# jacobwilliams/splpak

Hardware: AMD Instinct MI355X
Metric: fitted points/sec (splcw) + evals/sec (splfe), 3-D 1e7 pts 64^3 nodes (higher is better)
Workload: dtype f64; 1 GPU; C3: 3-D splcw least-squares spline fit, 10000000 weighted scattered points (Park-Miller stream, seed 42), 64x64x64 nodes, xtrap=1, real64; ncol=262144, points_per_gpu=10000000, points_total=10000000, parallelism=single GPU, rccl_ranks=0, refine_steps=2

## Files before the change

splpak_amd/csrc/ndchol.hip:

```cpp
#include "ndstate.hpp"
#include <cstdlib>

namespace splpak {
namespace nd {

hipError_t nd_prefit(splpak_plan *p, hipStream_t st, void *user)
{
    NdState *s = static_cast<NdState *>(user);
    s->tail_pending = false;
    if (s->sch.staged_init && !s->dist) return hipSuccess;
    if (!s->str.sU || !s->ev.evPre || splpak::opt_get("SPLPAK_ND_NO_EARLY_CLEAR")) return hipSuccess;
    long long head = 0;
    if (p->gscratch == s->factor) head = p->gscratch_doubles < s->factor_doubles ? p->gscratch_doubles : s->factor_doubles;
    else if (p->gscratch >= s->factor && p->gscratch < s->factor + s->factor_doubles) return hipSuccess;
    if (head >= s->factor_doubles) return hipSuccess;
    hipError_t e = hipEventRecord(s->ev.evPre, st);
    if (e == hipSuccess) e = hipStreamWaitEvent(s->str.sU, s->ev.evPre, 0);
    const int clear_wgs = splpak::opt_get("SPLPAK_ND_CLEAR_WGS") ? atoi(splpak::opt_get("SPLPAK_ND_CLEAR_WGS")) : 128;
    if (e == hipSuccess) {
        if (clear_wgs > 0) {
            launch_clear(clear_wgs, s->factor + head, s->factor_doubles - head, s->str.sU);
            e = hipGetLastError();
        } else
            e = hipMemsetAsync(s->factor + head, 0, sizeof(double) * (size_t)(s->factor_doubles - head), s->str.sU);
    }
    if (e == hipSuccess) e = hipEventRecord(s->ev.evTail, s->str.sU);
    if (e != hipSuccess) return e;
    s->tail_pending = true;
    s->head_doubles = head;
    return hipSuccess;
}

hipError_t nd_assemble(splpak_plan *p, hipStream_t st, void *user)
{
    NdState *s = static_cast<NdState *>(user);
    hipError_t e = hipSuccess;
    if (s->sch.staged_init && !s->dist) {
        if (!s->sch.istarts.empty())
            for (int x : s->sch.istarts[0]) launch_init(s, p->g, p->nst, s->fac.init.l[(size_t)x][0], st);
        return hipGetLastError();
    }
    if (s->tail_pending) {
        if (s->head_doubles > 0) e = hipMemsetAsync(s->factor, 0, sizeof(double) * (size_t)s->head_doubles, st);
        if (e == hipSuccess) e = hipStreamWaitEvent(st, s->ev.evTail, 0);
        s->tail_pending = false;
    } else
        e = hipMemsetAsync(s->factor, 0, sizeof(double) * (size_t)s->factor_doubles, st);
    if (e != hipSuccess) return e;
    launch_assemble(s, p->g, p->nst, st);
    return hipGetLastError();
}

namespace {

struct FactorRun {
    splpak_plan *p;
    NdState *s;
    hipStream_t st, sP, sU, sR;
    int *info_dev;
    double *minpiv_dev;
    CholStats *stats;
    bool timing;
    int pin_rounds;
    int qnext = 0;
    int la_evt = -1;
    bool joined = false, comm_failed = false;
    void syrk(const JobTable<SyrkJob> &tab, const Launch &l, hipStream_t q, bool schur, bool pinned) { launch_syrk(s, tab, l, q, stats, timing, schur, pinned, qnext); }
    void begin();
    void dist_join();
    void potrf_step(const Launch &lp, int k, hipStream_t sC, bool reserved, hipEvent_t after);
    void stage_prep(int i);
    void chain_step(int stg, int k, bool pinned, bool pin_potrf, int prep);
    void root_stage(int stg);
    void run_stage(int i);
    hipError_t end();
};

void hop(hipEvent_t e, hipStream_t from, hipStream_t to) { (void)hipEventRecord(e, from); (void)hipStreamWaitEvent(to, e, 0); }

void zero_block(NdState *s, int x, hipStream_t q) { launch_zero(s->fac.zero, s->fac.zero.l[(size_t)x][0], q); }

void ensure_events(NdState *s, int steps)
{
    for (auto *v : {&s->ev.evT, &s->ev.evI, &s->ev.evW})
        while ((int)v->size() < steps) v->push_back(nd_event(s));
}

void FactorRun::begin()
{
    NdTree &t = s->t;
    if (timing) {
        if (!s->ev.f0) { s->ev.f0 = nd_event(s, true); s->ev.f1 = nd_event(s, true); }
        (void)hipEventRecord(s->ev.f0, st);
    }
    if (s->used && s->ev.evDone) (void)hipStreamWaitEvent(st, s->ev.evDone, 0);
    if (s->zlast_valid) (void)hipStreamWaitEvent(st, s->ev.evZlast, 0);
    if (!s->s_clean && !s->sch.sc.st.empty())
        for (int x : s->sch.starts[0]) zero_block(s, x, st);
    s->s_clean = false;
    if (s->queues) (void)hipMemsetAsync(s->queues, 0, sizeof(int) * ND_QSTRIDE * (size_t)s->nqueues, st);
    if (s->dist && s->sh.rank != 0)
        for (int id : t.by_depth[(size_t)(s->sh.dcut - 1)]) {
            const NdFront &f = t.fr[(size_t)id];
            (void)hipMemsetAsync(s->factor + s->poff[(size_t)id], 0, sizeof(double) * (size_t)(f.ld * f.wp), st);
        }
    (void)hipEventRecord(s->ev.ev0, st);
    for (hipStream_t q : {sP, sU})
        if (q != st) (void)hipStreamWaitEvent(q, s->ev.ev0, 0);
    if (sR) (void)hipStreamWaitEvent(sR, s->ev.ev0, 0);
}

void FactorRun::dist_join()
{
    NdTree &t = s->t;
    joined = true;
    for (hipStream_t q : {sP, sU, sR})
        if (q) (void)hipStreamSynchronize(q);
    double *scratch = s->sh.join_scratch;
    long long scap = s->sh.join_scratch_doubles;
    if (!s->sch.sc.packed) {
        const double mine_missing = scratch ? 0.0 : 1.0;
        double any_missing = 0.0;
        (void)hipMemcpyAsync(s->part + 1, &mine_missing, sizeof(double), hipMemcpyHostToDevice, st);
        if (plan_allreduce(p, s->part + 1, 1, st) != 0) comm_failed = true;
        (void)hipMemcpyAsync(&any_missing, s->part + 1, sizeof(double), hipMemcpyDeviceToHost, st);
        (void)hipStreamSynchronize(st);
        if (any_missing != 0.0) scap = 0;
    }
    for (int id : t.by_depth[(size_t)(s->sh.dcut - 1)]) {
        const NdFront &f = t.fr[(size_t)id];
        if (plan_allreduce(p, s->factor + s->poff[(size_t)id], f.ld * (long long)f.wp, st) != 0) comm_failed = true;
        if (f.hp == 0) continue;
        const int nt = f.hp / 64;
        const long long tiles = trapezoid_items(nt, nt);
        if (s->sch.sc.packed) {
            if (plan_allreduce(p, s_ptr(s, id), nd_schur_doubles(f, true), st) != 0) comm_failed = true;
        } else if (tiles * 4096 <= scap) {
            launch_tripack(true, s_ptr(s, id), f.lds, nt, scratch, st);
            if (plan_allreduce(p, scratch, tiles * 4096, st) != 0) comm_failed = true;
            launch_tripack(false, s_ptr(s, id), f.lds, nt, scratch, st);
        } else if (plan_allreduce(p, s_ptr(s, id), f.lds * (long long)f.hp, st) != 0)
            comm_failed = true;
    }
    (void)hipStreamSynchronize(st);
}

void FactorRun::potrf_step(const Launch &lp, int k, hipStream_t sC, bool reserved, hipEvent_t after)
{
    if (!reserved) { launch_potrf(s, s->fac.potrf, lp, sC, info_dev, minpiv_dev); return; }
    if (after) (void)hipStreamWaitEvent(sR, after, 0);
    else hop(s->ev.evR0, sC, sR);
    launch_potrf(s, s->fac.potrf, lp, sR, info_dev, minpiv_dev);
    hop(s->ev.evI[(size_t)k], sR, sC);
}

void FactorRun::stage_prep(int i)
{
    for (int x : s->sch.starts[(size_t)i]) zero_block(s, x, sU);
    if (s->sch.staged_init && !s->dist)
        for (int x : s->sch.istarts[(size_t)i]) {
            launch_init(s, p->g, p->nst, s->fac.init.l[(size_t)x][0], sU);
            if (s->sch.sc.st[(size_t)x].dep < 0 && sU != sP) (void)hipEventRecord(s->ev.evP[(size_t)x], sU);
        }
}

void FactorRun::chain_step(int stg, int k, bool pinned, bool pin_potrf, int prep)
{
    FactorTables &F = s->fac;
    const size_t S = (size_t)stg, K = (size_t)k;
    hipStream_t sC = sP;
    const Launch &ls = F.schur.l[S][K], &lf0 = F.fin[0].l[S][K], &lf1 = F.fin[1].l[S][K];
    const bool ahead = pinned && k > 0 && la_evt == k - 1;
    potrf_step(F.potrf.l[S][K], k, sC, pinned && (pin_potrf || ahead), ahead ? s->ev.evW[(size_t)(k - 1)] : nullptr);
    launch_trsm(F.trsm, F.trsm.l[S][K], sC);
    if (prep >= 0) {
        hop(s->ev.evU, sC, sU);
        stage_prep(prep);
    }
    if ((ls.count || lf0.count || lf1.count) && sU != sC) hop(s->ev.evT[K], sC, sU);
    syrk(F.upd, F.upd.l[S][K], sC, false, pinned);
    if (s->sch.chain_la[S] && F.updr.l[S][K].count) {
        if (pinned) {
            (void)hipEventRecord(s->ev.evW[K], sC);
            la_evt = k;
        }
        syrk(F.updr, F.updr.l[S][K], sC, false, pinned);
    }
    syrk(F.updo, F.updo.l[S][K], sC, false, pinned);
    syrk(F.schur, ls, sU, true, pinned);
    syrk(F.fin[0], lf0, sU, true, pinned);
    syrk(F.fin[1], lf1, sU, true, pinned);
}

void FactorRun::root_stage(int stg)
{
    FactorTables &F = s->fac;
    const size_t S = (size_t)stg;
    const int steps = (int)F.potrf.l[S].size();
    ensure_events(s, steps);
    const bool pinned = sR != nullptr && s->nres > 0 && steps > 0 && (int)F.potrf.l[S][0].grid <= pin_rounds * s->nres;
    const bool la = s->sch.lookahead[S] != 0, la2 = s->sch.lookahead[S] == 2;
    for (int k = 0; k < steps; ++k) {
        if (!la) { chain_step(stg, k, pinned, true, -1); continue; }
        const size_t K = (size_t)k;
        const Launch &ltb = F.trsmb.l[S][K], &lur = F.updr.l[S][K];
        potrf_step(F.potrf.l[S][K], k, sP, pinned, nullptr);
        if (ltb.count) {
            if (sU != sP) {
                if (!pinned) (void)hipEventRecord(s->ev.evI[K], sP);
                (void)hipStreamWaitEvent(sU, s->ev.evI[K], 0);
            }
            launch_trsm(F.trsmb, ltb, sU);
        }
        if (!la2 && k > 0 && sU != sP) (void)hipStreamWaitEvent(sP, s->ev.evW[K - 1], 0);
        launch_trsm(F.trsm, F.trsm.l[S][K], sP);
        if (lur.count && sU != sP) hop(s->ev.evT[K], sP, sU);
        if (la2 && k > 0 && sU != sP) (void)hipStreamWaitEvent(sP, s->ev.evW[K - 1], 0);
        syrk(F.upd, F.upd.l[S][K], sP, false, pinned);
        syrk(F.updr, lur, sU, false, pinned);
        if (sU != sP) (void)hipEventRecord(s->ev.evW[K], sU);
    }
    if (sU != sP) hop(s->ev.evU, sU, sP);
}

void FactorRun::run_stage(int i)
{
    FactorTables &F = s->fac;
    const NdStage &S = s->sch.sc.st[(size_t)i];
    if (s->dist && !joined && S.depth <= s->sh.dcut - 1) dist_join();
    auto passes = [&](int k) { return F.schur.l[(size_t)i][(size_t)k].count || F.fin[0].l[(size_t)i][(size_t)k].count || F.fin[1].l[(size_t)i][(size_t)k].count; };
    const int steps = (int)F.potrf.l[(size_t)i].size();
    const bool prep_late = splpak::opt_get("SPLPAK_ND_PREP_EARLY") == nullptr;
    const bool defer = prep_late && i > 0 && i != s->sch.root_stage && sU != sP && steps >= 2 && !passes(0);
    if (i > 0) {
        if (!defer) stage_prep(i);
        if (s->sch.staged_init && !s->dist && S.dep < 0 && sU != sP) (void)hipStreamWaitEvent(sP, s->ev.evP[(size_t)i], 0);
    }
    if (s->sch.fused && S.dep >= 0 && sU != sP) (void)hipStreamWaitEvent(sP, s->ev.evF[(size_t)S.dep], 0);
    la_evt = -1;
    if (i == s->sch.root_stage) { root_stage(i); return; }
    ensure_events(s, steps);
    const bool pinned = sR != nullptr && s->nres > 0 && steps > 0 && ((int)F.potrf.l[(size_t)i][0].grid <= pin_rounds * s->nres || s->sch.chain_la[(size_t)i]);
    const bool unpin_first = splpak::opt_get("SPLPAK_ND_PIN_FIRST") == nullptr;
    bool pass_running = !unpin_first;
    for (int k = 0; k < steps; ++k) {
        chain_step(i, k, pinned, pass_running, k == 0 && defer ? i : -1);
        if (passes(k)) pass_running = true;
    }
    if (s->sch.fused) (void)hipEventRecord(s->ev.evF[(size_t)i], sU);
    else {
        if (sU != sP) hop(s->ev.evU, sU, sP);
        for (int sl = 0; sl < 2; ++sl) launch_add(F.add, F.add.l[(size_t)i][(size_t)sl], sP);
        (void)hipEventRecord(s->ev.evE[(size_t)i], sP);
        if (sU != sP) (void)hipStreamWaitEvent(sU, s->ev.evE[(size_t)i], 0);
    }
}

hipError_t FactorRun::end()
{
    if (s->dist && !joined && s->sh.dcut >= 1) dist_join();
    hipError_t top_err = hipSuccess;
    if (s->mdist) {
        ++s->top.fgen;
        top_err = nd_top_factor(s, st, info_dev, minpiv_dev, stats, timing);
    }
    if (top_err == hipSuccess && !s->sch.sc.st.empty())
        for (int x : s->sch.starts[0]) zero_block(s, x, sU);
    launch_trinv(s->fac.trinv.dev, s->fac.ntrinv, sP);
    (void)hipEventRecord(s->ev.evJ, sP);
    if (sP != st) (void)hipStreamWaitEvent(st, s->ev.evJ, 0);
    if (s->mdist && top_err == hipSuccess) top_err = nd_top_pivots(s, st, info_dev, minpiv_dev);
    if (s->dist) {
        launch_flag(info_dev, s->part, st);
        if (plan_allreduce(p, s->part, 1, st) != 0) comm_failed = true;
        launch_unflag(info_dev, s->part, st);
    }
    if (sU != st) {
        (void)hipEventRecord(s->ev.evZlast, sU);
        s->zlast_valid = true;
    }
    s->s_clean = true;
    (void)hipEventRecord(s->ev.evDone, st);
    s->used = true;
    hipError_t err = hipGetLastError();
    if (timing) {
        (void)hipEventRecord(s->ev.f1, st);
        (void)hipEventSynchronize(s->ev.f1);
        float ms = 0;
        (void)hipEventElapsedTime(&ms, s->ev.f0, s->ev.f1);
        stats->factor_ms = ms;
        for (size_t i = 0; i < (size_t)stats->syrk_launches; ++i) {
            if (hipEventElapsedTime(&ms, s->ev.evA[i], s->ev.evB[i]) == hipSuccess) stats->syrk_ms += ms;
            else (void)hipGetLastError();
        }
    }
    if (err != hipSuccess || top_err != hipSuccess) s->s_clean = false;
    if (comm_failed) return hipErrorUnknown;
    return top_err != hipSuccess ? top_err : err;
}

}

hipError_t nd_factor(splpak_plan *p, int *info_dev, double *minpiv_dev, hipStream_t st, void *user)
{
    NdState *s = static_cast<NdState *>(user);
    const bool timing = p->stats.enabled;
    p->stats = CholStats{};
    p->stats.enabled = timing;
    const bool serial = splpak::opt_get("SPLPAK_NO_LOOKAHEAD") != nullptr;
    FactorRun r{p, s, st, s->str.sP, s->str.sU, s->str.sR, info_dev, minpiv_dev, &p->stats, timing};
    if (serial) r.sP = r.sU = st;
    if (serial || splpak::opt_get("SPLPAK_NO_PANEL_CU")) r.sR = nullptr;
    r.pin_rounds = splpak::opt_get("SPLPAK_ND_PIN_ROUNDS") ? atoi(splpak::opt_get("SPLPAK_ND_PIN_ROUNDS")) : 1;
    r.begin();
    for (int i = 0; i < (int)s->sch.sc.st.size(); ++i) r.run_stage(i);
    return r.end();
}

hipError_t nd_solve(splpak_plan *p, double *x, double *tmp, hipStream_t st, void *user)
{
    (void)tmp;
    NdState *s = static_cast<NdState *>(user);
    NdTree &t = s->t;
    SolveTables &T = s->sol;
    const long long n = t.vec_doubles;
    launch_gather(n, s->rowsrc, x, s->V, st);
    bool comm_failed = false;
    if (s->dist && s->sh.rank != 0)
        for (int id : t.by_depth[(size_t)(s->sh.dcut - 1)]) {
            const NdFront &f = t.fr[(size_t)id];
            (void)hipMemsetAsync(s->V + f.vofs, 0, sizeof(double) * (size_t)f.fp, st);
        }
    const int dlow = s->mdist ? s->top.pt.dcut : 0;
    if (s->mdist) ++s->top.sgen;
    for (int d = t.maxdepth; d >= dlow; --d) {
        if (d < t.maxdepth)
            for (int sl = 0; sl < 2; ++sl) launch_map(T.map, T.map.l[(size_t)(d + 1)][(size_t)sl], false, st);
        if (s->dist && d == s->sh.dcut - 1)
            for (int id : t.by_depth[(size_t)d]) {
                const NdFront &f = t.fr[(size_t)id];
                if (plan_allreduce(p, s->V + f.vofs, f.fp, st) != 0) comm_failed = true;
            }
        const int steps = (int)T.mv.l[(size_t)d].size();
        for (int k = 0; k < steps; ++k) {
            launch_mv(T.mv, T.mv.l[(size_t)d][(size_t)k], st);
            launch_fwd(T.fwd, T.fwd.l[(size_t)d][(size_t)k], st);
        }
    }
    if (s->mdist) {
        hipError_t e = nd_top_forward(s, st);
        if (e == hipSuccess) e = nd_top_backward(s, st);
        if (e != hipSuccess) return e;
    }
    for (int d = dlow; d <= t.maxdepth; ++d) {
        if (d >= 1 && d > dlow) launch_map(T.map, T.map.l[(size_t)d][2], true, st);
        const int steps = (int)T.mv.l[(size_t)d].size();
        for (int k = steps - 1; k >= 0; --k) {
            launch_dot(T.dot, T.dot.l[(size_t)d][(size_t)k], st);
            launch_bwd(T.bwd, T.bwd.l[(size_t)d][(size_t)k], st);
        }
    }
    if (s->dist || s->mdist) {
        (void)hipMemsetAsync(x, 0, sizeof(double) * (size_t)p->g.ncol, st);
        launch_scatter(n, s->sh.rowsrc_out, s->V, x, st);
        if (plan_allreduce(p, x, p->g.ncol, st) != 0) comm_failed = true;
    } else
        launch_scatter(n, s->rowsrc, s->V, x, st);
    if (comm_failed) return hipErrorUnknown;
    return hipGetLastError();
}

}
}
```

splpak_amd/csrc/ndjobs.hip:

```cpp
#include "ndstate.hpp"
#include <algorithm>

namespace splpak {
namespace nd {

namespace {

void front_step_jobs(NdState *s, int stg, int id, int k, bool two_level)
{
    NdTree &t = s->t;
    FactorTables &F = s->fac;
    const NdFront &f = t.fr[(size_t)id];
    const bool la = s->sch.lookahead[(size_t)stg] != 0, la2 = s->sch.lookahead[(size_t)stg] == 2, cla = s->sch.chain_la[(size_t)stg] != 0;
    const int schur_kb = s->sch.schur_kb;
    const int g0 = (k / schur_kb) * schur_kb, gend = std::min(g0 + schur_kb, f.nsteps) - 1;
    double *panel = s->factor + s->poff[(size_t)id];
    double *diag = panel + (long long)k * 256 + (long long)k * 256 * f.ld;
    double *below = diag + 256;
    const int nrows = f.fp - (k + 1) * 256;
    double *i16 = s->inv16 + (long long)(s->lblk[(size_t)id] + k) * 4096;
    const int ncols = std::max(1, std::min(256, f.w - k * 256));
    F.potrf.push(PotrfJob{diag, i16, f.ld, f.own0 + k * 256, ncols});
    const int nc = (f.wp - (k + 1) * 256) / 64, nr = nrows / 64;
    if (nrows > 0) {
        const int ntop = (la && !la2 && nc > 0) ? std::min(nrows, 256) : nrows;
        F.trsm.push(TrsmJob{diag, below, i16, f.ld, ntop, 0, (ncols + 15) / 16, 0}, ntop / 16);
        if (nrows > ntop) F.trsmb.push(TrsmJob{diag, below + ntop, i16, f.ld, nrows - ntop, 0, (ncols + 15) / 16, 0}, (nrows - ntop) / 16);
    }
    if (nc > 0) {
        const SyrkJob proto{below, below + (long long)256 * f.ld, f.ld, f.ld, 0, 0, 0, 1, 64, 0, nullptr, nullptr, nullptr, 0, 0, 0, 0};
        auto trapezoid = [&](JobTable<SyrkJob> &tab, int c, int r) {
            SyrkJob a = proto;
            a.nc = c; a.nr = r;
            tab.push(a, trapezoid_items(c, r));
        };
        auto split = [&](JobTable<SyrkJob> &rect_tab, int nin) {
            const int n4 = std::min(nin, 4);
            trapezoid(F.upd, n4, std::min(nr, 4));
            if (nr > 4) {
                SyrkJob r = proto;
                r.nc = n4; r.nr = nr; r.zinit = -4;
                rect_tab.push(r, (long long)n4 * (nr - 4));
            }
            if (nin > 4) {
                SyrkJob t2 = proto;
                t2.P = below + 256;
                t2.C = below + (long long)256 * f.ld + 256 + (long long)256 * f.ld;
                t2.nc = nin - 4; t2.nr = nr - 4;
                F.updr.push(t2, trapezoid_items(nin - 4, nr - 4));
            }
        };
        if (!la && two_level) {
            const int nc_in = std::min(nc, (gend - k) * 4);
            if (nc_in > 0 && cla) split(F.updr, nc_in);
            else if (nc_in > 0) trapezoid(F.upd, nc_in, nr);
            if (k == gend) {
                SyrkJob o = proto;
                o.P = panel + (long long)(k + 1) * 256 + (long long)g0 * 256 * f.ld;
                o.kb = k - g0 + 1;
                o.nc = nc; o.nr = nr;
                F.updo.push(o, trapezoid_items(nc, nr));
                F.updo.cur.flop += 2.0 * 64 * 64 * 256.0 * o.kb * (double)trapezoid_items(nc, nr);
            }
        } else if (!la)
            trapezoid(F.upd, nc, nr);
        else
            split(la2 ? F.upd : F.updr, nc);
    }
    const int ns = f.hp / 64;
    if (ns > 0 && k == gend) {
        const int kb = k - g0 + 1;
        const int ksl = (k == f.nsteps - 1) ? 4 * ((ncols + 15) / 16) : 64;
        const double jitems = (double)trapezoid_items(ns, ns) - (s->full_diag ? 0.0 : 0.375 * ns);
        const double jflop = 2.0 * 64 * 64 * (256.0 * (kb - 1) + 4.0 * ksl) * jitems;
        const bool boundary = s->mdist && f.depth == s->top.pt.dcut;
        if (s->sch.fused && k == f.nsteps - 1 && f.parent >= 0 && !boundary) {
            const NdFront &pf = t.fr[(size_t)f.parent];
            const int leaf = s->sch.needs[(size_t)id] ? 0 : 1;
            F.fin[f.slot].push(SyrkJob{panel + f.wp + (long long)g0 * 256 * f.ld, s_ptr(s, id), f.ld, s_ld(s, id), ns, ns, 0, kb, ksl, leaf, s->pmap + f.bofs,
                                       s->factor + s->poff[(size_t)f.parent], s_ptr(s, f.parent), pf.ld, s_ld(s, f.parent), pf.wp, f.h},
                               trapezoid_items(ns, ns));
            F.fin[f.slot].cur.flop += jflop;
        } else {
            F.schur.push(SyrkJob{panel + f.wp + (long long)g0 * 256 * f.ld, s_ptr(s, id), f.ld, s_ld(s, id), ns, ns, 0, kb, ksl, 0, nullptr, nullptr, nullptr, 0, 0, 0, 0},
                         trapezoid_items(ns, ns));
            F.schur.cur.flop += jflop;
        }
    }
}

bool stage_jobs(NdState *s, int stg)
{
    NdTree &t = s->t;
    FactorTables &F = s->fac;
    const std::vector<int> &ids = s->sch.sc.st[(size_t)stg].ids;
    F.zero.open();
    for (int id : ids) {
        const NdFront &f = t.fr[(size_t)id];
        if (f.hp == 0 || !s->sch.needs[(size_t)id]) continue;
        const int nt = f.hp / 64;
        F.zero.push(ZeroJob{s_ptr(s, id), s_ld(s, id), nt, 0}, trapezoid_items(nt, nt));
    }
    if (!F.zero.close((size_t)stg, 0)) return false;
    F.init.open();
    for (int id : ids)
        if (s->poff[(size_t)id] >= 0) F.init.push(InitJob{id, 0}, t.fr[(size_t)id].wp);
    if (!F.init.close((size_t)stg, 0)) return false;
    if (s->sch.sc.st[(size_t)stg].depth >= 1 && !s->sch.fused)
        for (int sl = 0; sl < 2; ++sl) {
            F.add.open();
            for (int id : ids) {
                const NdFront &f = t.fr[(size_t)id];
                if (f.slot != sl || f.h == 0) continue;
                const NdFront &p = t.fr[(size_t)f.parent];
                const int nt = f.hp / 64;
                F.add.push(AddJob{s_ptr(s, id), s->pmap + f.bofs, s->factor + s->poff[(size_t)f.parent], s_ptr(s, f.parent), s_ld(s, id), p.ld,
                                  s_ld(s, f.parent), f.h, nt, p.wp, 0},
                           trapezoid_items(nt, nt));
            }
            if (!F.add.close((size_t)stg, (size_t)sl)) return false;
        }
    return true;
}

bool nd_build_factor_jobs(NdState *s)
{
    NdTree &t = s->t;
    FactorTables &F = s->fac;
    const int nstage = (int)s->sch.sc.st.size();
    JobTable<SyrkJob> *const syrk[] = {&F.upd, &F.updr, &F.updo, &F.schur, &F.fin[0], &F.fin[1]};
    s->sch.lookahead.assign((size_t)nstage, 0);
    s->sch.chain_la.assign((size_t)nstage, 0);
    for_each_table(F, [&](auto &tab) { tab.l.assign((size_t)nstage, {}); });
    const bool two_level = splpak::opt_get("SPLPAK_ND_NO_OUTER") == nullptr;
    for (int stg = 0; stg < nstage; ++stg) {
        const std::vector<int> &ids = s->sch.sc.st[(size_t)stg].ids;
        int steps = 0;
        for (int id : ids) steps = std::max(steps, t.fr[(size_t)id].nsteps);
        bool any_schur = false;
        for (int id : ids) any_schur = any_schur || t.fr[(size_t)id].hp > 0;
        const bool la = !any_schur && steps >= 4 && !splpak::opt_get("SPLPAK_ND_NO_ROOT_LOOKAHEAD");
        const bool la2 = la && !(splpak::opt_get("SPLPAK_ND_ROOT_LA") && atoi(splpak::opt_get("SPLPAK_ND_ROOT_LA")) == 1);
        const int cla_blocks = splpak::opt_get("SPLPAK_ND_CHAIN_LA") ? atoi(splpak::opt_get("SPLPAK_ND_CHAIN_LA")) : 8;
        const bool cla = !la && two_level && steps >= 2 && (int)ids.size() <= cla_blocks && !s->mdist;
        s->sch.chain_la[(size_t)stg] = cla ? 1 : 0;
        s->sch.lookahead[(size_t)stg] = la ? (la2 ? 2 : 1) : 0;
        for (int k = 0; k < steps; ++k) {
            F.potrf.open(); F.trsm.open(); F.trsmb.open();
            for (auto *tab : syrk) tab->open();
            for (int id : ids)
                if (k < t.fr[(size_t)id].nsteps) front_step_jobs(s, stg, id, k, two_level);
            const size_t S = (size_t)stg, K = (size_t)k;
            if (!F.potrf.close(S, K) || !F.trsm.close(S, K) || !F.trsmb.close(S, K)) return false;
            for (auto *tab : syrk)
                if (!tab->close(S, K)) return false;
            F.upd.l[S][K].flop = 2.0 * 64 * 64 * 256 * (double)F.upd.l[S][K].grid;
            F.updr.l[S][K].flop = 2.0 * 64 * 64 * 256 * (double)F.updr.l[S][K].grid;
        }
        if (!stage_jobs(s, stg)) return false;
    }
    for (size_t id = 0; id < t.fr.size(); ++id) {
        const NdFront &f = t.fr[id];
        if (!s->mine.empty() && !s->mine[id]) continue;
        for (int k = 0; k < f.nsteps; ++k) {
            const double *diag = s->factor + s->poff[id] + (long long)k * 256 + (long long)k * 256 * f.ld;
            const long long lb = s->lblk[id] + k;
            F.trinv.host.push_back(TrinvJob{diag, s->inv16 + lb * 4096, s->dinv + lb * 65536, s->dinvt + lb * 65536, f.ld});
        }
    }
    F.ntrinv = (int)F.trinv.host.size();
    return true;
}

bool nd_build_solve_jobs(NdState *s)
{
    NdTree &t = s->t;
    SolveTables &T = s->sol;
    const int nd = t.maxdepth + 1;
    for_each_table(T, [&](auto &tab) { tab.l.assign((size_t)nd, {}); });
    long long part_max = 0;
    for (int d = 0; d < nd; ++d) {
        std::vector<int> ids;
        for (int id : t.by_depth[(size_t)d])
            if (s->mine.empty() || s->mine[(size_t)id]) ids.push_back(id);
        int steps = 0;
        for (int id : ids) steps = std::max(steps, t.fr[(size_t)id].nsteps);
        for (int k = 0; k < steps; ++k) {
            T.mv.open(); T.fwd.open(); T.dot.open(); T.bwd.open();
            long long partofs = 0;
            for (int id : ids) {
                const NdFront &f = t.fr[(size_t)id];
                if (k >= f.nsteps) continue;
                const double *below = s->factor + s->poff[(size_t)id] + (long long)k * 256 + (long long)k * 256 * f.ld + 256;
                const int nrows = f.fp - (k + 1) * 256;
                double *Vf = s->V + f.vofs, *Yf = s->Y + f.vofs;
                T.mv.push(MvJob{s->dinv + (long long)(s->lblk[(size_t)id] + k) * 65536, Vf + k * 256, Yf + k * 256});
                int nsplit = 0;
                double *partp = s->part + partofs;
                if (nrows > 0) {
                    T.fwd.push(FwdJob{below, Yf + k * 256, Vf + (k + 1) * 256, f.ld, nrows, 0}, nrows / 64);
                    nsplit = (nrows + DOT_RPS - 1) / DOT_RPS;
                    T.dot.push(DotJob{below, Vf + (k + 1) * 256, partp, f.ld, nrows, nsplit, DOT_RPS, 0}, 16 * nsplit);
                    partofs += (long long)nsplit * 256;
                }
                T.bwd.push(BwdJob{s->dinvt + (long long)(s->lblk[(size_t)id] + k) * 65536, Yf + k * 256, partp, Vf + k * 256, nsplit, 0});
            }
            part_max = std::max(part_max, partofs);
            const size_t D = (size_t)d, K = (size_t)k;
            if (!T.mv.close(D, K) || !T.fwd.close(D, K) || !T.dot.close(D, K) || !T.bwd.close(D, K)) return false;
        }
        if (d >= 1) {
            for (int sl = 0; sl < 2; ++sl) {
                T.map.open();
                for (int id : ids) {
                    const NdFront &f = t.fr[(size_t)id];
                    if (f.slot != sl || f.h == 0) continue;
                    const NdFront &p = t.fr[(size_t)f.parent];
                    T.map.push(MapJob{s->V + f.vofs + f.wp, s->V + p.vofs, s->pmap + f.bofs, f.h, 0});
                }
                if (!T.map.close((size_t)d, (size_t)sl)) return false;
            }
            const int first = T.map.l[(size_t)d][0].first, both = T.map.l[(size_t)d][0].count + T.map.l[(size_t)d][1].count;
            T.map.l[(size_t)d].push_back(Launch{first, both, (unsigned)both, 0});
        }
    }
    return part_max <= s->part_cap;
}

}

int nd_make_jobs(NdState *s)
{
    auto each = [&](auto &&f) { for_each_table(s->fac, f); for_each_table(s->sol, f); };
    each([](auto &tab) { tab.host.clear(); });
    if (!nd_build_factor_jobs(s) || !nd_build_solve_jobs(s)) return SPLPAK_E_UNSUPPORTED;
    bool ok = true;
    each([&](auto &tab) { nd_free_dev(s, &tab.dev); ok = ok && nd_upload(s, &tab.dev, tab.host); });
    return ok ? 0 : SPLPAK_E_NOMEM;
}

bool nd_build_top_jobs(NdState *s)
{
    NdGroup *g = s->grp;
    NdTree &t = s->t;
    Top &T = s->top;
    const NdPartition &pt = T.pt;
    const int me = s->mrank, nseq = pt.nseq;
    const size_t ntop = pt.top.size();
    for_each_table(T, [&](auto &tab) { tab.l.assign(1, std::vector<Launch>((size_t)nseq + 1)); });
    T.rslot.assign((size_t)nseq + 1, -1);
    for (int sl = 0; sl < 2; ++sl) {
        T.l_pull[sl].assign(ntop, Launch());
        T.l_mapf[sl].assign(ntop, -1);
// ... 123 lines not shown
```

splpak_amd/csrc/ndstate.hpp:

```cpp
#pragma once
#include "plan.hpp"
#include "ndtree.hpp"
#include <atomic>
#include <memory>
#include <string>
#include <vector>

namespace splpak {

struct NdGroup {
    int R = 1, chunk = 1;
    std::vector<void *> st;
    std::atomic<int> *abort = nullptr;
    std::atomic<int> own_abort{0};
    HostBarrier bar;
    int nseq = 0;
    std::unique_ptr<std::atomic<int>[]> posted, fposted, bposted, subdone;
    std::vector<int> h_info;
    std::vector<double> h_minpiv;
    bool finalized = false;
    int gen = 0;
};

namespace nd {

struct PotrfJob { double *A; double *inv16; long long ld; int k0; int ncols; };
struct TrsmJob { const double *L; double *X; const double *inv16; long long ld; int nrows; int wg0; int ncb; int pad; };
struct SyrkJob {
    const double *P; double *C; long long ldp, ldc; int nc, nr; int item0; int kb; int ksl; int zinit;
    const int *pm; double *Pp; double *Sp; long long ldpp, ldsp; int wpp; int h;
};
struct ZeroJob { double *S; long long lds; int nt; int tile0; };
struct InitJob { int front; int col0; };
struct TrinvJob { const double *L; const double *inv16; double *dinv; double *dinvt; long long ld; };
struct AddJob { const double *S; const int *pm; double *P; double *Sp; long long lds, ldp, ldsp; int h, nt, wpp, tile0; };
struct MvJob { const double *M; const double *v; double *out; };
struct FwdJob { const double *L; const double *y; double *v; long long ld; int nrows; int wg0; };
struct DotJob { const double *L; const double *x; double *part; long long ld; int nrows; int nsplit; int rps; int wg0; };
struct BwdJob { const double *Mt; const double *y; const double *part; double *x; int nsplit; int pad; };
struct MapJob { double *child; double *par; const int *pm; int h; int pad; };
struct FrontDev { long long panel_off, ld, bofs; int own0, w, wp, h; int top; int pad; };
struct TopColDev { long long off, ld; };
struct PullJob { const double *src; long long lds; const int *pm; double *dst; long long ldd; int c0, c1, h, row0, tile0, ntr, ntc, pad; };

constexpr int DOT_RPS = 1024;
constexpr int ND_QSTRIDE = 16;

inline int *first_item(TrsmJob &j) { return &j.wg0; }
inline int *first_item(SyrkJob &j) { return &j.item0; }
inline int *first_item(ZeroJob &j) { return &j.tile0; }
inline int *first_item(InitJob &j) { return &j.col0; }
inline int *first_item(AddJob &j) { return &j.tile0; }
inline int *first_item(FwdJob &j) { return &j.wg0; }
inline int *first_item(DotJob &j) { return &j.wg0; }
inline int *first_item(PullJob &j) { return &j.tile0; }
template <typename J> inline int *first_item(J &) { return nullptr; }
template <typename J> inline J end_job(const J *) { return J{}; }
inline InitJob end_job(const InitJob *) { return InitJob{-1, 0}; }

struct Launch { int first = 0, count = 0; unsigned grid = 0; double flop = 0; };

template <typename J>
struct JobTable {
    std::vector<J> host;
    J *dev = nullptr;
    std::vector<std::vector<Launch>> l;
    Launch cur;
    long long items = 0;

    void open() { cur = Launch(); cur.first = (int)host.size(); items = 0; }
    void push(J j, long long n = 1)
    {
        if (int *f = first_item(j)) *f = (int)items;
        host.push_back(j);
        items += n;
        ++cur.count;
    }
    bool close(Launch &out, bool sentinel = true)
    {
        if (items > 0x7fffffffLL) { set_error("nested dissection: launch too large"); return false; }
        cur.grid = (unsigned)items;
        J e = end_job((const J *)nullptr);
        if (int *f = first_item(e); f && sentinel && cur.count) { *f = (int)items; host.push_back(e); }
        out = cur;
        return true;
    }
    bool close(size_t r, size_t c, bool sentinel = true)
    {
        if (l[r].size() <= c) l[r].resize(c + 1);
        return close(l[r][c], sentinel);
    }
};

struct FactorTables {
    JobTable<PotrfJob> potrf;
    JobTable<TrsmJob> trsm, trsmb;
    JobTable<SyrkJob> upd;
    JobTable<SyrkJob> updr;
    JobTable<SyrkJob> updo;
    JobTable<SyrkJob> fin[2];
    JobTable<SyrkJob> schur;
    JobTable<TrinvJob> trinv;
    JobTable<AddJob> add;
    JobTable<ZeroJob> zero;
    JobTable<InitJob> init;
    int ntrinv = 0;
};
template <typename F> void for_each_table(FactorTables &T, F &&f)
{
    f(T.potrf); f(T.trsm); f(T.trsmb); f(T.upd); f(T.updr); f(T.updo); f(T.fin[0]); f(T.fin[1]); f(T.schur); f(T.trinv); f(T.add); f(T.zero); f(T.init);
}

struct SolveTables {
    JobTable<MvJob> mv;
    JobTable<FwdJob> fwd;
    JobTable<DotJob> dot;
    JobTable<BwdJob> bwd;
    JobTable<MapJob> map;
};
template <typename F> void for_each_table(SolveTables &T, F &&f) { f(T.mv); f(T.fwd); f(T.dot); f(T.bwd); f(T.map); }

struct Schedule {
    NdSchedule sc;
    std::vector<char> needs;
    std::vector<std::vector<int>> starts;
    std::vector<std::vector<int>> istarts;
    int root_stage = -1;
    int schur_kb = 4;
    std::vector<char> lookahead;
    std::vector<char> chain_la;
    bool fused = true;
    bool staged_init = false;
};

struct Streams {
    hipStream_t sP = nullptr, sU = nullptr, sR = nullptr, sCopy = nullptr;
};

struct Events {
    std::vector<hipEvent_t> all;
    hipEvent_t ev0 = nullptr, evJ = nullptr, evU = nullptr, evZlast = nullptr, evDone = nullptr, evPre = nullptr, evTail = nullptr, evR0 = nullptr;
    hipEvent_t f0 = nullptr, f1 = nullptr;
    std::vector<hipEvent_t> evF;
    std::vector<hipEvent_t> evE;
    std::vector<hipEvent_t> evP;
    std::vector<hipEvent_t> evI;
    std::vector<hipEvent_t> evT;
    std::vector<hipEvent_t> evW;
    std::vector<hipEvent_t> evA, evB;
};

struct Shard {
    int world = 1, rank = 0, dcut = 0;
    double *join_scratch = nullptr;
    long long join_scratch_doubles = 0;
    int *rowsrc_out = nullptr;
};

struct Top {
    NdPartition pt;
    std::vector<long long> tbase;
    std::vector<TopColDev> topcol;
    std::vector<int> toplblk;
    TopColDev *topcol_dev = nullptr;
    double *pbuf[3] = {nullptr, nullptr, nullptr};
    double *stagev = nullptr;
    long long stagev_doubles = 0;
    JobTable<PotrfJob> potrf;
    JobTable<TrsmJob> trsm;
    JobTable<SyrkJob> chain, bulk;
    JobTable<PullJob> pull;
    JobTable<TrinvJob> trinv;
    JobTable<MvJob> mv;
    JobTable<FwdJob> fwd;
    JobTable<DotJob> dot;
    JobTable<BwdJob> bwd;
    JobTable<MapJob> mapf, mapb, maps;
    std::vector<Launch> l_pull[2];
    std::vector<int> l_mapf[2], l_mapb, l_maps;
    std::vector<int> subroots;
    std::vector<int> rslot;
    std::vector<hipEvent_t> evReady, evArr, evCol, evBulk, evSF, evSB, evAdd;
    hipEvent_t evSub = nullptr, evTop = nullptr;
    int fgen = 0, sgen = 0;
};
template <typename F> void for_each_table(Top &T, F &&f)
{
    f(T.potrf); f(T.trsm); f(T.chain); f(T.bulk); f(T.pull); f(T.trinv); f(T.mv); f(T.fwd); f(T.dot); f(T.bwd); f(T.mapf); f(T.mapb); f(T.maps);
}

struct NdState {
    NdTree t;
    int device = 0;
    std::string desc;
    double *factor = nullptr, *dinv = nullptr, *dinvt = nullptr, *inv16 = nullptr;
    long long factor_doubles = 0;
    int nblocks = 0;
    std::vector<char> mine;
    std::vector<long long> poff;
    std::vector<int> lblk;
    double *sarena = nullptr;
    long long sarena_doubles = 0;
    double *V = nullptr, *Y = nullptr, *part = nullptr;
    long long part_cap = 0;
    int *pos = nullptr, *front_of = nullptr, *bpos = nullptr, *pmap = nullptr, *rowsrc = nullptr;
    int *ipos = nullptr;
    std::vector<int> rowsrc_host;
    long long *padwhere = nullptr;
    int npad = 0;
    FrontDev *fdev = nullptr;
    std::vector<void *> owned;
    size_t owned_bytes = 0;
    unsigned *resmap = nullptr;
    int nres = 0;
    int potrf_waves = 8;
    int xmode = 1;
    int full_diag = 0;
    bool small_queue = false;
    int wg4 = 0;
    int small_grid = 1024;
    int *queues = nullptr;
    int nqueues = 0;
    Schedule sch;
    FactorTables fac;
    SolveTables sol;
    Streams str;
    Events ev;
    bool dist = false;
    Shard sh;
    bool mdist = false;
    NdGroup *grp = nullptr;
// ... 75 lines not shown
```

splpak_amd/csrc/options.hip:

```cpp
#include "options.hpp"

#include <cctype>
#include <cstdlib>
#include <cstring>
#include <mutex>

extern char **environ;

namespace splpak {

namespace {
struct Known { const char *name; int documented; };
const Known KNOWN[] = {
    {"SPLPAK_BIN_ATOMIC", 0},
    {"SPLPAK_DEBUG", 1},
    {"SPLPAK_DEBUG_NO_PEER", 0},
    {"SPLPAK_DEBUG_SUMS", 0},
    {"SPLPAK_DEBUG_TWOEND", 0},
    {"SPLPAK_DIST_CHUNK", 0},
    {"SPLPAK_GRAM_SCRATCH_MB", 1},
    {"SPLPAK_GRAM_VALU", 0},
    {"SPLPAK_MPLAN_BAND", 0},
    {"SPLPAK_MPLAN_RCCL", 1},
    {"SPLPAK_NARROW_BW", 0},
    {"SPLPAK_ND", 1},
    {"SPLPAK_ND_CHAIN_LA", 0},
    {"SPLPAK_ND_CHUNK", 0},
    {"SPLPAK_ND_CLEAR_WGS", 0},
    {"SPLPAK_ND_CUT", 1},
    {"SPLPAK_ND_DIST", 0},
    {"SPLPAK_ND_FULL_DIAG", 0},
    {"SPLPAK_ND_HALVES", 0},
    {"SPLPAK_ND_KB", 1},
    {"SPLPAK_ND_NO_EARLY_CLEAR", 0},
    {"SPLPAK_ND_NO_FUSE", 0},
    {"SPLPAK_ND_NO_OUTER", 0},
    {"SPLPAK_ND_NO_ROOT_LOOKAHEAD", 0},
    {"SPLPAK_ND_PIN_FIRST", 0},
    {"SPLPAK_ND_PIN_ROUNDS", 0},
    {"SPLPAK_ND_POTRF_WAVES", 0},
    {"SPLPAK_ND_PREP_EARLY", 0},
    {"SPLPAK_ND_RES_CUS", 1},
    {"SPLPAK_ND_ROOT_LA", 0},
    {"SPLPAK_ND_SMALL_GRID", 0},
    {"SPLPAK_ND_SMALL_QUEUE", 0},
    {"SPLPAK_ND_SPLIT", 1},
    {"SPLPAK_ND_SQUARE", 0},
    {"SPLPAK_ND_STAGED_INIT", 0},
    {"SPLPAK_ND_WG4", 0},
    {"SPLPAK_ND_XCD", 0},
    {"SPLPAK_NO_LOOKAHEAD", 0},
    {"SPLPAK_NO_PANEL_CU", 0},
    {"SPLPAK_NO_PLAN_CACHE", 1},
    {"SPLPAK_NO_REORDER", 1},
    {"SPLPAK_NO_TWOEND", 0},
    {"SPLPAK_PCG_ALWAYS", 0},
    {"SPLPAK_PCG_ASSEMBLE", 0},
    {"SPLPAK_PCG_EAGER", 0},
    {"SPLPAK_PCG_MAXIT", 1},
    {"SPLPAK_PCG_NO_BLOCKS", 0},
    {"SPLPAK_PCG_NO_PAIRS", 0},
    {"SPLPAK_PCG_PAIRS_VALU", 0},
    {"SPLPAK_PCG_TOL1", 1},
    {"SPLPAK_PCG_TOL2", 1},
    {"SPLPAK_PIN_BW", 0},
    {"SPLPAK_RCCL_JOB", 0},
    {"SPLPAK_RCCL_LIB", 1},
    {"SPLPAK_RCCL_ONE_RANK_CALLS", 0},
    {"SPLPAK_RESIDUAL_CELLS", 0},
    {"SPLPAK_ROWS_ONE_STREAM", 0},
    {"SPLPAK_ROWS_TILES", 0},
    {"SPLPAK_SOLVER", 1},
    {"SPLPAK_VIRTUAL_GPUS", 0},
};
std::mutex g_mu;
std::map<std::string, std::string> g_defaults;
thread_local const Options *t_current = nullptr;
thread_local Options t_fallback;
thread_local unsigned long long t_fallback_gen = ~0ull;
unsigned long long g_gen = 0;
}

bool option_canonical(const char *name, std::string &canon)
{
    if (!name) return false;
    std::string s(name);
    for (char &c : s) c = (char)std::toupper((unsigned char)c);
    if (s.rfind("SPLPAK_", 0) != 0) s = "SPLPAK_" + s;
    for (const Known &k : KNOWN)
        if (s == k.name) { canon = s; return true; }
    return false;
}

Options options_snapshot()
{
    Options o;
    for (char **e = environ; e && *e; ++e) {
        if (std::strncmp(*e, "SPLPAK_", 7) != 0) continue;
        const char *eq = std::strchr(*e, '=');
        if (!eq) continue;
        o.kv[std::string(*e, (size_t)(eq - *e))] = std::string(eq + 1);
    }
    std::lock_guard<std::mutex> lk(g_mu);
    for (const auto &d : g_defaults) o.kv[d.first] = d.second;
    return o;
}

int options_set_default(const char *name, const char *value)
{
    std::string canon;
    if (!option_canonical(name, canon)) return -1;
    std::lock_guard<std::mutex> lk(g_mu);
    ++g_gen;
    if (value) g_defaults[canon] = value;
    else g_defaults.erase(canon);
    return 0;
}

const char *opt_get(const char *canon)
{
    if (t_current) return t_current->get(canon);
    unsigned long long gen;
    {
        std::lock_guard<std::mutex> lk(g_mu);
        gen = g_gen;
        auto d = g_defaults.find(canon);
        if (d != g_defaults.end()) {
            if (t_fallback_gen != gen) { t_fallback.kv.clear(); t_fallback_gen = gen; }
            t_fallback.kv[canon] = d->second;
            return t_fallback.kv[canon].c_str();
        }
// ... 9 lines not shown
```

Baseline: 40.66 million points/s.

## Add deeper root look-ahead, pinned group stages, and per-stage triangular inverses

Adds a third root look-ahead form that splits each step's trailing update into a small critical corner (upd), a near-panel column band (updc) and the far remainder (updr). This lets the next potrf wait only on the corner update, through a new per-step event, instead of the whole trailing update. It also pins more multi-step stages to the reserved compute units, and launches triangular-inverse jobs per stage right after each stage factors rather than in one tail batch. A host-side coverage check verifies the split tiles exactly once; the costs are more launches and more event traffic.

```diff
diff --git a/splpak_amd/csrc/ndchol.hip b/splpak_amd/csrc/ndchol.hip
--- a/splpak_amd/csrc/ndchol.hip
+++ b/splpak_amd/csrc/ndchol.hip
@@ -53,6 +53,8 @@
 
 namespace {
 
+constexpr bool PIN_GROUPS_DEFAULT = true, TRINV_STAGED_DEFAULT = true;
+
 struct FactorRun {
     splpak_plan *p;
     NdState *s;
@@ -62,6 +64,8 @@
     CholStats *stats;
     bool timing;
     int pin_rounds;
+    bool pin_groups = false;
+    bool trinv_staged = false;
     int qnext = 0;
     int la_evt = -1;
     bool joined = false, comm_failed = false;
@@ -82,7 +86,7 @@
 
 void ensure_events(NdState *s, int steps)
 {
-    for (auto *v : {&s->ev.evT, &s->ev.evI, &s->ev.evW})
+    for (auto *v : {&s->ev.evT, &s->ev.evI, &s->ev.evW, &s->ev.evD})
         while ((int)v->size() < steps) v->push_back(nd_event(s));
 }
 
@@ -199,11 +203,25 @@
     const int steps = (int)F.potrf.l[S].size();
     ensure_events(s, steps);
     const bool pinned = sR != nullptr && s->nres > 0 && steps > 0 && (int)F.potrf.l[S][0].grid <= pin_rounds * s->nres;
-    const bool la = s->sch.lookahead[S] != 0, la2 = s->sch.lookahead[S] == 2;
+    const bool la = s->sch.lookahead[S] != 0, la2 = s->sch.lookahead[S] == 2, la3 = s->sch.lookahead[S] == 3;
     for (int k = 0; k < steps; ++k) {
         if (!la) { chain_step(stg, k, pinned, true, -1); continue; }
         const size_t K = (size_t)k;
         const Launch &ltb = F.trsmb.l[S][K], &lur = F.updr.l[S][K];
+        if (la3) {
+            const bool ahead = pinned && k > 0 && F.upd.l[S][K - 1].count != 0;
+            potrf_step(F.potrf.l[S][K], k, sP, pinned, ahead ? s->ev.evD[K - 1] : nullptr);
+            launch_trsm(F.trsm, F.trsm.l[S][K], sP);
+            syrk(F.upd, F.upd.l[S][K], sP, false, pinned);
+            if (pinned && F.upd.l[S][K].count) (void)hipEventRecord(s->ev.evD[K], sP);
+            launch_trsm(F.trsmb, ltb, sP);
+            if (lur.count && sU != sP) hop(s->ev.evT[K], sP, sU);
+            if (k > 0 && sU != sP) (void)hipStreamWaitEvent(sP, s->ev.evW[K - 1], 0);
+            syrk(F.updc, F.updc.l[S][K], sP, false, pinned);
+            syrk(F.updr, lur, sU, false, pinned);
+            if (sU != sP) (void)hipEventRecord(s->ev.evW[K], sU);
+            continue;
+        }
         potrf_step(F.potrf.l[S][K], k, sP, pinned, nullptr);
         if (ltb.count) {
             if (sU != sP) {
@@ -240,13 +258,16 @@
     la_evt = -1;
     if (i == s->sch.root_stage) { root_stage(i); return; }
     ensure_events(s, steps);
-    const bool pinned = sR != nullptr && s->nres > 0 && steps > 0 && ((int)F.potrf.l[(size_t)i][0].grid <= pin_rounds * s->nres || s->sch.chain_la[(size_t)i]);
+    const bool pinned = sR != nullptr && s->nres > 0 && steps > 0 &&
+                        ((int)F.potrf.l[(size_t)i][0].grid <= pin_rounds * s->nres || s->sch.chain_la[(size_t)i] ||
+                         (pin_groups && steps > s->sch.schur_kb && (int)F.potrf.l[(size_t)i][0].grid <= 2 * s->nres));
     const bool unpin_first = splpak::opt_get("SPLPAK_ND_PIN_FIRST") == nullptr;
     bool pass_running = !unpin_first;
     for (int k = 0; k < steps; ++k) {
         chain_step(i, k, pinned, pass_running, k == 0 && defer ? i : -1);
         if (passes(k)) pass_running = true;
     }
+    if (trinv_staged) launch_trinv(F.trinv.dev + F.trinv.l[(size_t)i][0].first, F.trinv.l[(size_t)i][0].count, sP);
     if (s->sch.fused) (void)hipEventRecord(s->ev.evF[(size_t)i], sU);
     else {
         if (sU != sP) hop(s->ev.evU, sU, sP);
@@ -266,7 +287,8 @@
     }
     if (top_err == hipSuccess && !s->sch.sc.st.empty())
         for (int x : s->sch.starts[0]) zero_block(s, x, sU);
-    launch_trinv(s->fac.trinv.dev, s->fac.ntrinv, sP);
+    if (trinv_staged) launch_trinv(s->fac.trinv.dev + s->fac.trinv_tail.first, s->fac.trinv_tail.count, sP);
+    else launch_trinv(s->fac.trinv.dev, s->fac.ntrinv, sP);
     (void)hipEventRecord(s->ev.evJ, sP);
     if (sP != st) (void)hipStreamWaitEvent(st, s->ev.evJ, 0);
     if (s->mdist && top_err == hipSuccess) top_err = nd_top_pivots(s, st, info_dev, minpiv_dev);
@@ -312,6 +334,9 @@
     if (serial) r.sP = r.sU = st;
     if (serial || splpak::opt_get("SPLPAK_NO_PANEL_CU")) r.sR = nullptr;
     r.pin_rounds = splpak::opt_get("SPLPAK_ND_PIN_ROUNDS") ? atoi(splpak::opt_get("SPLPAK_ND_PIN_ROUNDS")) : 1;
+    auto on = [](const char *name, bool dflt) { const char *v = splpak::opt_get(name); return v ? atoi(v) != 0 : dflt; };
+    r.pin_groups = on("SPLPAK_ND_PIN_GROUPS", PIN_GROUPS_DEFAULT);
+    r.trinv_staged = on("SPLPAK_ND_TRINV_STAGED", TRINV_STAGED_DEFAULT) && !s->mdist && !s->dist;
     r.begin();
     for (int i = 0; i < (int)s->sch.sc.st.size(); ++i) r.run_stage(i);
     return r.end();
diff --git a/splpak_amd/csrc/ndjobs.hip b/splpak_amd/csrc/ndjobs.hip
--- a/splpak_amd/csrc/ndjobs.hip
+++ b/splpak_amd/csrc/ndjobs.hip
@@ -11,7 +11,8 @@
     NdTree &t = s->t;
     FactorTables &F = s->fac;
     const NdFront &f = t.fr[(size_t)id];
-    const bool la = s->sch.lookahead[(size_t)stg] != 0, la2 = s->sch.lookahead[(size_t)stg] == 2, cla = s->sch.chain_la[(size_t)stg] != 0;
+    const bool la = s->sch.lookahead[(size_t)stg] != 0, la2 = s->sch.lookahead[(size_t)stg] == 2, la3 = s->sch.lookahead[(size_t)stg] == 3;
+    const bool cla = s->sch.chain_la[(size_t)stg] != 0;
     const int schur_kb = s->sch.schur_kb;
     const int g0 = (k / schur_kb) * schur_kb, gend = std::min(g0 + schur_kb, f.nsteps) - 1;
     double *panel = s->factor + s->poff[(size_t)id];
@@ -64,7 +65,24 @@
             }
         } else if (!la)
             trapezoid(F.upd, nc, nr);
-        else
+        else if (la3) {
+            auto sub = [&](JobTable<SyrkJob> &tab, int o, int c, int r) {
+                SyrkJob a = proto;
+                a.P = below + 64 * o;
+                a.C = proto.C + (long long)64 * o * (f.ld + 1);
+                a.nc = c; a.nr = r;
+                tab.push(a, trapezoid_items(c, r));
+            };
+            const int n4 = std::min(nc, 4);
+            sub(F.upd, 0, n4, std::min(nr, 4));
+            if (nr > 4) {
+                SyrkJob r = proto;
+                r.nc = n4; r.nr = nr; r.zinit = -4;
+                F.updc.push(r, (long long)n4 * (nr - 4));
+            }
+            if (nc > 4) sub(F.updc, 4, std::min(nc - 4, 4), nr - 4);
+            if (nc > 8) sub(F.updr, 8, nc - 8, nr - 8);
+        } else
             split(la2 ? F.upd : F.updr, nc);
     }
     const int ns = f.hp / 64;
@@ -89,6 +107,29 @@
     }
 }
 
+std::string cover_check(const std::vector<const SyrkJob *> &jobs, const double *P0, const double *C0, long long ld, int nc, int nr)
+{
+    std::vector<int> seen((size_t)std::max(nc, 0) * (size_t)std::max(nr, 0), 0);
+    for (const SyrkJob *j : jobs) {
+        const long long off = j->C - C0, pofs = j->P - P0;
+        if (off < 0 || pofs < 0 || j->ldc != ld || j->ldp != ld) return "a job outside the trailing matrix";
+        if (pofs % 64 || off % ld != pofs || off / ld != pofs) return "a job whose tiles and panel rows disagree";
+        const int o = (int)(pofs / 64);
+        const int rb = j->zinit < 0 ? -j->zinit : 0;
+        if (rb && j->nc > rb) return "a rectangle wider than its first row";
+        for (int tj = 0; tj < j->nc; ++tj)
+            for (int ti = rb ? rb : tj; ti < j->nr; ++ti) {
+                const int ci = o + ti, cj = o + tj;
+                if (ci >= nr || cj >= nc) return "a tile outside the trailing trapezoid";
+                if (++seen[(size_t)cj * (size_t)nr + (size_t)ci] > 1) return "a tile updated twice";
+            }
+    }
+    for (int tj = 0; tj < nc; ++tj)
+        for (int ti = tj; ti < nr; ++ti)
+            if (!seen[(size_t)tj * (size_t)nr + (size_t)ti]) return "a tile no job updates";
+    return std::string();
+}
+
 bool stage_jobs(NdState *s, int stg)
 {
     NdTree &t = s->t;
@@ -123,12 +164,28 @@
     return true;
 }
 
+constexpr int ROOT_LA_DEFAULT = 3;
+
+bool step_covered(NdState *s, int id, int k)
+{
+    FactorTables &F = s->fac;
+    const NdFront &f = s->t.fr[(size_t)id];
+    const double *below = s->factor + s->poff[(size_t)id] + (long long)k * 256 + (long long)k * 256 * f.ld + 256;
+    std::vector<const SyrkJob *> jobs;
+    for (auto *tab : {&F.upd, &F.updc, &F.updr})
+        for (int j = 0; j < tab->cur.count; ++j) jobs.push_back(&tab->host[(size_t)(tab->cur.first + j)]);
+    const std::string msg = cover_check(jobs, below, below + (long long)256 * f.ld, f.ld, (f.wp - (k + 1) * 256) / 64, (f.fp - (k + 1) * 256) / 64);
+    if (msg.empty()) return true;
+    set_error("nested dissection: root look-ahead, block step " + std::to_string(k) + ": " + msg);
+    return false;
+}
+
 bool nd_build_factor_jobs(NdState *s)
 {
     NdTree &t = s->t;
     FactorTables &F = s->fac;
     const int nstage = (int)s->sch.sc.st.size();
-    JobTable<SyrkJob> *const syrk[] = {&F.upd, &F.updr, &F.updo, &F.schur, &F.fin[0], &F.fin[1]};
+    JobTable<SyrkJob> *const syrk[] = {&F.upd, &F.updr, &F.updc, &F.updo, &F.schur, &F.fin[0], &F.fin[1]};
     s->sch.lookahead.assign((size_t)nstage, 0);
     s->sch.chain_la.assign((size_t)nstage, 0);
     for_each_table(F, [&](auto &tab) { tab.l.assign((size_t)nstage, {}); });
@@ -140,11 +197,13 @@
         bool any_schur = false;
         for (int id : ids) any_schur = any_schur || t.fr[(size_t)id].hp > 0;
         const bool la = !any_schur && steps >= 4 && !splpak::opt_get("SPLPAK_ND_NO_ROOT_LOOKAHEAD");
-        const bool la2 = la && !(splpak::opt_get("SPLPAK_ND_ROOT_LA") && atoi(splpak::opt_get("SPLPAK_ND_ROOT_LA")) == 1);
+        const char *la_opt = splpak::opt_get("SPLPAK_ND_ROOT_LA");
+        const int la_form = !la ? 0 : ((la_opt && atoi(la_opt) >= 1 && atoi(la_opt) <= 3) ? atoi(la_opt) : ROOT_LA_DEFAULT);
+        const int la_val = (la_form == 3 && (s->mdist || s->dist)) ? 2 : la_form;
         const int cla_blocks = splpak::opt_get("SPLPAK_ND_CHAIN_LA") ? atoi(splpak::opt_get("SPLPAK_ND_CHAIN_LA")) : 8;
         const bool cla = !la && two_level && steps >= 2 && (int)ids.size() <= cla_blocks && !s->mdist;
         s->sch.chain_la[(size_t)stg] = cla ? 1 : 0;
-        s->sch.lookahead[(size_t)stg] = la ? (la2 ? 2 : 1) : 0;
+        s->sch.lookahead[(size_t)stg] = (char)la_val;
         for (int k = 0; k < steps; ++k) {
             F.potrf.open(); F.trsm.open(); F.trsmb.open();
             for (auto *tab : syrk) tab->open();
@@ -154,21 +213,34 @@
             if (!F.potrf.close(S, K) || !F.trsm.close(S, K) || !F.trsmb.close(S, K)) return false;
             for (auto *tab : syrk)
                 if (!tab->close(S, K)) return false;
-            F.upd.l[S][K].flop = 2.0 * 64 * 64 * 256 * (double)F.upd.l[S][K].grid;
-            F.updr.l[S][K].flop = 2.0 * 64 * 64 * 256 * (double)F.updr.l[S][K].grid;
+            for (auto *tab : {&F.upd, &F.updr, &F.updc}) tab->l[S][K].flop = 2.0 * 64 * 64 * 256 * (double)tab->l[S][K].grid;
+            if (la && ids.size() == 1 && !step_covered(s, ids[0], k)) return false;
         }
         if (!stage_jobs(s, stg)) return false;
     }
-    for (size_t id = 0; id < t.fr.size(); ++id) {
+    std::vector<char> listed(t.fr.size(), 0);
+    auto front_inverses = [&](size_t id) {
         const NdFront &f = t.fr[id];
-        if (!s->mine.empty() && !s->mine[id]) continue;
+        if (listed[id] || (!s->mine.empty() && !s->mine[id])) return;
+        listed[id] = 1;
         for (int k = 0; k < f.nsteps; ++k) {
             const double *diag = s->factor + s->poff[id] + (long long)k * 256 + (long long)k * 256 * f.ld;
             const long long lb = s->lblk[id] + k;
             F.trinv.host.push_back(TrinvJob{diag, s->inv16 + lb * 4096, s->dinv + lb * 65536, s->dinvt + lb * 65536, f.ld});
         }
-    }
+    };
+    for (int stg = 0; stg < nstage; ++stg) {
+        Launch l;
+        l.first = (int)F.trinv.host.size();
+        if (stg != s->sch.root_stage)
+            for (int id : s->sch.sc.st[(size_t)stg].ids) front_inverses((size_t)id);
+        l.count = (int)F.trinv.host.size() - l.first;
+        F.trinv.l[(size_t)stg].assign(1, l);
+    }
+    F.trinv_tail.first = (int)F.trinv.host.size();
+    for (size_t id = 0; id < t.fr.size(); ++id) front_inverses(id);
     F.ntrinv = (int)F.trinv.host.size();
+    F.trinv_tail.count = F.ntrinv - F.trinv_tail.first;
     return true;
 }
 
diff --git a/splpak_amd/csrc/ndstate.hpp b/splpak_amd/csrc/ndstate.hpp
--- a/splpak_amd/csrc/ndstate.hpp
+++ b/splpak_amd/csrc/ndstate.hpp
@@ -97,10 +97,12 @@
     JobTable<TrsmJob> trsm, trsmb;
     JobTable<SyrkJob> upd;
     JobTable<SyrkJob> updr;
+    JobTable<SyrkJob> updc;
     JobTable<SyrkJob> updo;
     JobTable<SyrkJob> fin[2];
     JobTable<SyrkJob> schur;
     JobTable<TrinvJob> trinv;
+    Launch trinv_tail;
     JobTable<AddJob> add;
     JobTable<ZeroJob> zero;
     JobTable<InitJob> init;
@@ -108,7 +110,7 @@
 };
 template <typename F> void for_each_table(FactorTables &T, F &&f)
 {
-    f(T.potrf); f(T.trsm); f(T.trsmb); f(T.upd); f(T.updr); f(T.updo); f(T.fin[0]); f(T.fin[1]); f(T.schur); f(T.trinv); f(T.add); f(T.zero); f(T.init);
+    f(T.potrf); f(T.trsm); f(T.trsmb); f(T.upd); f(T.updr); f(T.updc); f(T.updo); f(T.fin[0]); f(T.fin[1]); f(T.schur); f(T.trinv); f(T.add); f(T.zero); f(T.init);
 }
 
 struct SolveTables {
@@ -147,6 +149,7 @@
     std::vector<hipEvent_t> evI;
     std::vector<hipEvent_t> evT;
     std::vector<hipEvent_t> evW;
+    std::vector<hipEvent_t> evD;
     std::vector<hipEvent_t> evA, evB;
 };
 
diff --git a/splpak_amd/csrc/options.hip b/splpak_amd/csrc/options.hip
--- a/splpak_amd/csrc/options.hip
+++ b/splpak_amd/csrc/options.hip
@@ -37,6 +37,7 @@
     {"SPLPAK_ND_NO_OUTER", 0},
     {"SPLPAK_ND_NO_ROOT_LOOKAHEAD", 0},
     {"SPLPAK_ND_PIN_FIRST", 0},
+    {"SPLPAK_ND_PIN_GROUPS", 0},
     {"SPLPAK_ND_PIN_ROUNDS", 0},
     {"SPLPAK_ND_POTRF_WAVES", 0},
     {"SPLPAK_ND_PREP_EARLY", 0},
@@ -47,6 +48,7 @@
     {"SPLPAK_ND_SPLIT", 1},
     {"SPLPAK_ND_SQUARE", 0},
     {"SPLPAK_ND_STAGED_INIT", 0},
+    {"SPLPAK_ND_TRINV_STAGED", 0},
     {"SPLPAK_ND_WG4", 0},
     {"SPLPAK_ND_XCD", 0},
     {"SPLPAK_NO_LOOKAHEAD", 0},
```

After: 40.73 million points/s (median of 3 runs). About the same (+0.2%).
